# SeanNaren/deepspeech.pytorch

Measured on NVIDIA H100. Metric: utterances/sec (train step, 161x1000 spectrogram), higher is better.
Workload: dtype fp16-operands(rnn)+tf32(conv/fc)

## Files before the change

deepspeech.pytorch_b200/_lib.py:

```python
import ctypes as C
import os

_HERE = os.path.dirname(os.path.abspath(__file__))
LIB_PATH = os.path.join(_HERE, "libds2_b200.so")

RNN_LSTM, RNN_GRU, RNN_TANH = 0, 1, 2
PREC_FP32, PREC_TF32, PREC_F16 = 0, 1, 2

vp, i32, i64, f32, sz = C.c_void_p, C.c_int, C.c_int64, C.c_float, C.c_size_t


class RnnDesc(C.Structure):
    _fields_ = [("rnn_type", i32), ("bidirectional", i32), ("T", i32), ("B", i32), ("In", i32), ("H", i32),
                ("training", i32), ("bn_momentum", f32), ("bn_eps", f32), ("deferred_dw", i32)]


PROTOTYPES = {
    "ds2_version": (C.c_char_p, []),
    "ds2_last_error": (C.c_char_p, []),
    "ds2_device_check": (i32, [C.POINTER(i32)] * 3),
    "ds2_set_precision": (i32, [i32]),
    "ds2_get_precision": (i32, []),
    "ds2_launch_count": (i64, [i32]),
    "ds2_fallback_count": (i64, [i32]),
    "ds2_set_side_stream": (i32, [vp]),
    "ds2_join_side_stream": (i32, [vp]),
    "ds2_prof_enable": (i32, [i32]),
    "ds2_prof_report": (i32, [C.c_char_p, sz]),
    "ds2_seq_lens_host": (i32, [vp, i32, vp]),
    "ds2_conv_frontend_workspace_bytes": (sz, [i32, i32]),
    "ds2_conv_frontend_fwd": (i32, [i32, i32] + [vp] * 14 + [i32, f32, f32] + [vp] * 6 + [sz, vp]),
    "ds2_conv_frontend_bwd": (i32, [i32, i32] + [vp] * 22 + [sz, vp]),
    "ds2_rnn_reserve_floats": (sz, [C.POINTER(RnnDesc)]),
    "ds2_rnn_workspace_bytes": (sz, [C.POINTER(RnnDesc)]),
    "ds2_rnn_layer_fwd": (i32, [C.POINTER(RnnDesc)] + [vp] * 17 + [sz, vp]),
    "ds2_rnn_layer_bwd": (i32, [C.POINTER(RnnDesc)] + [vp] * 18 + [sz, vp]),
    "ds2_lookahead_fwd": (i32, [i32] * 4 + [vp] * 4),
    "ds2_lookahead_bwd": (i32, [i32] * 4 + [vp] * 7),
    "ds2_fc_head_workspace_bytes": (sz, [i32, i32, i32]),
    "ds2_fc_head_fwd": (i32, [i32, i32, i32] + [vp] * 6 + [i32, f32, f32, i32] + [vp] * 4 + [sz, vp]),
    "ds2_fc_head_bwd": (i32, [i32, i32, i32] + [vp] * 11 + [sz, vp]),
    "ds2_ctc_workspace_bytes": (sz, [i32, i32, i32, i32]),
    "ds2_ctc_loss_fwd_bwd": (i32, [i32, i32, i32] + [vp] * 4 + [i32, i32] + [vp] * 3 + [sz, vp]),
    "ds2_greedy_decode": (i32, [i32, i32, i32, vp, vp, i32, vp, vp, vp, vp]),
    "ds2_spectrogram_workspace_bytes": (sz, [i32]),
    "ds2_spectrogram_batch": (i32, [i32, vp, vp, vp, i32, i32, i32, vp, i32, i32, vp, i32, vp, sz, vp]),
    "ds2_spec_augment_workspace_bytes": (sz, [i32]),
    "ds2_spec_augment": (i32, [i32, i32, i32] + [vp] * 5 + [sz, vp]),
    "ds2_optim_workspace_bytes": (sz, []),
    "ds2_adamw_step": (i32, [i64] + [vp] * 4 + [f32] * 5 + [i32, f32, f32, vp, vp, vp]),
    "ds2_sgd_nesterov_step": (i32, [i64] + [vp] * 3 + [f32] * 3 + [i32, f32, f32, vp, vp, vp]),
    "ds2_gemm_workspace_bytes": (sz, [i32] * 5),
    "ds2_gemm": (i32, [i32] * 5 + [f32, vp, i32, vp, i32, f32, vp, i32, vp, sz, vp]),
    "ds2_gemm_f16": (i32, [i32] * 3 + [f32, vp, i32, vp, i32, f32, vp, i32, vp]),
}

_lib = None


class Ds2Error(RuntimeError):
    pass


def get_lib():
    global _lib
    if _lib is None:
        if not os.path.exists(LIB_PATH):
            raise Ds2Error(f"{LIB_PATH} not found: build it with `make -C deepspeech.pytorch_b200/csrc` "
                           "(or __graft_entry__.build()); there is no CPU / eager fallback")
        import torch
        lib = C.CDLL(LIB_PATH)
        for name, (res, args) in PROTOTYPES.items():
            fn = getattr(lib, name)
            fn.restype, fn.argtypes = res, args
        _lib = lib
    return _lib


def check(rc, what=""):
    if rc != 0:
        msg = get_lib().ds2_last_error().decode(errors="replace")
        raise Ds2Error(f"{what} failed with code {rc}: {msg}")


def ptr(t):
    return None if t is None else C.c_void_p(t.data_ptr())


def ptr_array(tensors):
    arr = (C.c_void_p * len(tensors))(*[None if t is None else t.data_ptr() for t in tensors])
    return arr
```

deepspeech.pytorch_b200/csrc/gemm_simt.cu:

```cuda
#include "common.cuh"

namespace ds2 {

constexpr int BM = 128, BN = 128, BK = 16, TM = 8, TN = 8;

template <bool TA, bool TB>
__global__ void __launch_bounds__(256) gemm_simt_kernel(int M, int N, int K, float alpha,
                                                        const float* __restrict__ A, int lda,
                                                        const float* __restrict__ B, int ldb, float beta,
                                                        float* __restrict__ C, int ldc, int k_per_split,
                                                        float* __restrict__ part) {
  __shared__ __align__(16) float As[BK][BM + 4];
  __shared__ __align__(16) float Bs[BK][BN + 4];
  const int tid = threadIdx.x;
  const int m0 = blockIdx.y * BM, n0 = blockIdx.x * BN;
  const int tx = tid % 16, ty = tid / 16;
  float acc[TM][TN];
#pragma unroll
  for (int i = 0; i < TM; ++i)
#pragma unroll
    for (int j = 0; j < TN; ++j) acc[i][j] = 0.f;

  const int k_begin = blockIdx.z * k_per_split;
  const int k_end = min(K, k_begin + k_per_split);
// ... 85 lines not shown
  const int kps = cdiv(cdiv(K, splits), BK) * BK, gz = cdiv(K, kps);
  if (gz > 1) *k_per_split = kps;
  return gz;
}
size_t gemm_simt_workspace_bytes(int M, int N, int K) {
  int kps;
  const int gz = simt_splits(M, N, K, &kps);
  return gz > 1 ? (size_t)gz * M * N * sizeof(float) : 0;
}

int gemm_simt(int transA, int transB, int M, int N, int K, float alpha, const float* A, int lda, const float* B,
              int ldb, float beta, float* C, int ldc, cudaStream_t st, void* ws, size_t ws_bytes) {
  if (M <= 0 || N <= 0) return DS2_OK;
  dim3 grid(cdiv(N, BN), cdiv(M, BM));
  int k_per_split;
  const int gz = simt_splits(M, N, K, &k_per_split);
  float* part = nullptr;
  if (gz > 1 && ws && ws_bytes >= (size_t)gz * M * N * sizeof(float)) {
    grid.z = gz;
    part = static_cast<float*>(ws);
  } else {
    k_per_split = K > 0 ? K : 1;
  }
  if (transA) {
    if (transB) DS2_LAUNCH((gemm_simt_kernel<true, true>), grid, 256, 0, st, M, N, K, alpha, A, lda, B, ldb, beta, C, ldc, k_per_split, part);
    else DS2_LAUNCH((gemm_simt_kernel<true, false>), grid, 256, 0, st, M, N, K, alpha, A, lda, B, ldb, beta, C, ldc, k_per_split, part);
  } else {
    if (transB) DS2_LAUNCH((gemm_simt_kernel<false, true>), grid, 256, 0, st, M, N, K, alpha, A, lda, B, ldb, beta, C, ldc, k_per_split, part);
    else DS2_LAUNCH((gemm_simt_kernel<false, false>), grid, 256, 0, st, M, N, K, alpha, A, lda, B, ldb, beta, C, ldc, k_per_split, part);
  }
  if (part) DS2_LAUNCH(sum_splits_kernel, cdiv((long long)M * N, 256), 256, 0, st, M, N, gz, part, beta, C, ldc);
  return DS2_OK;
}

}

extern "C" {
size_t ds2_gemm_workspace_bytes(int transA, int transB, int M, int N, int K) {
  const size_t tc = ds2::gemm_tc_workspace_bytes(transA, transB, M, N, K), simt = ds2::gemm_simt_workspace_bytes(M, N, K);
  return tc > simt ? tc : simt;
}

int ds2_gemm(int transA, int transB, int M, int N, int K, float alpha, const float* A, int lda, const float* B,
             int ldb, float beta, float* C, int ldc, void* ws, size_t ws_bytes, void* stream) {
  DS2_REQUIRE(M >= 0 && N >= 0 && K >= 0 && A && B && C, "ds2_gemm: bad arguments");
  cudaStream_t st = ds2::as_stream(stream);
  if (ds2::tensor_core_mode()) {
    int r = ds2::gemm_tc(transA, transB, M, N, K, alpha, A, lda, B, ldb, beta, C, ldc, ws, ws_bytes, st);
    if (r <= 0) return r;
  }
  return ds2::gemm_simt(transA, transB, M, N, K, alpha, A, lda, B, ldb, beta, C, ldc, st, ws, ws_bytes);
}

int ds2_gemm_f16(int M, int N, int K, float alpha, const void* A16, int lda, const void* B16, int ldb, float beta,
                 float* C, int ldc, void* stream) {
  DS2_REQUIRE(M > 0 && N > 0 && K > 0 && A16 && B16 && C, "ds2_gemm_f16: bad arguments");
  int r = ds2::gemm_tc_f16(M, N, K, alpha, A16, lda, B16, ldb, beta, C, ldc, nullptr, ds2::as_stream(stream));
  DS2_REQUIRE(r != 1, "ds2_gemm_f16: shape %dx%dx%d / alignment not eligible for the fp16 tensor-core kernel", M, N, K);
  return r;
}
}
```

deepspeech.pytorch_b200/csrc/gemm_tc.cu:

```cuda
#include <stdio.h>
#include <stdlib.h>

#include "common.cuh"
#include "tc_common.cuh"

namespace ds2 {

typedef CUresult (*EncodeTiledFn)(CUtensorMap*, CUtensorMapDataType, cuuint32_t, void*, const cuuint64_t*,
                                  const cuuint64_t*, const cuuint32_t*, const cuuint32_t*, CUtensorMapInterleave,
                                  CUtensorMapSwizzle, CUtensorMapL2promotion, CUtensorMapFloatOOBfill);
static EncodeTiledFn g_encode = nullptr;
static CUtensorMapDataType g_tmap_dtype = CU_TENSOR_MAP_DATA_TYPE_TFLOAT32;

static int load_encode() {
  if (g_encode) return DS2_OK;
  void* fn = nullptr;
  cudaDriverEntryPointQueryResult q;
  DS2_CHECK_CUDA(cudaGetDriverEntryPoint("cuTensorMapEncodeTiled", &fn, cudaEnableDefault, &q));
  if (!fn || q != cudaDriverEntryPointSuccess) {
    set_error("cuTensorMapEncodeTiled not available from the driver");
    return DS2_ERR_CUDA;
  }
  const char* e = getenv("DS2_TMAP_TF32");
  if (e && e[0] == '0') g_tmap_dtype = CU_TENSOR_MAP_DATA_TYPE_FLOAT32;
// ... 55 lines not shown
  if (rc) return rc;
  cuuint64_t gdim[5], gstr[4];
  cuuint32_t bx[5], estr[5];
  for (int i = 0; i < rank; ++i) { gdim[i] = dims[i]; bx[i] = box[i]; estr[i] = 1; }
  for (int i = 0; i + 1 < rank; ++i) gstr[i] = strides_bytes[i];
  CUresult r = g_encode(out, g_tmap_dtype, (cuuint32_t)rank, const_cast<float*>(base), gdim, gstr, bx, estr,
                        CU_TENSOR_MAP_INTERLEAVE_NONE, CU_TENSOR_MAP_SWIZZLE_128B, CU_TENSOR_MAP_L2_PROMOTION_L2_256B,
                        CU_TENSOR_MAP_FLOAT_OOB_FILL_NONE);
  if (r != CUDA_SUCCESS) {
    set_error("cuTensorMapEncodeTiled(rank %d) failed: %d", rank, (int)r);
    return DS2_ERR_CUDA;
  }
  return DS2_OK;
}

int make_tmap_4d_f32(CUtensorMap* out, const float* base, const unsigned long long dims[4],
                     const unsigned long long strides_bytes[3], const unsigned int box[4]) {
  int rc = load_encode();
  if (rc) return rc;
  cuuint64_t gdim[4] = {dims[0], dims[1], dims[2], dims[3]};
  cuuint64_t gstr[3] = {strides_bytes[0], strides_bytes[1], strides_bytes[2]};
  cuuint32_t bx[4] = {box[0], box[1], box[2], box[3]};
  cuuint32_t estr[4] = {1, 1, 1, 1};
  CUresult r = g_encode(out, g_tmap_dtype, 4, const_cast<float*>(base), gdim, gstr, bx, estr,
                        CU_TENSOR_MAP_INTERLEAVE_NONE, CU_TENSOR_MAP_SWIZZLE_128B, CU_TENSOR_MAP_L2_PROMOTION_L2_256B,
                        CU_TENSOR_MAP_FLOAT_OOB_FILL_NONE);
  if (r != CUDA_SUCCESS) {
    set_error("cuTensorMapEncodeTiled(4d %llu,%llu,%llu,%llu) failed: %d", dims[0], dims[1], dims[2], dims[3], (int)r);
    return DS2_ERR_CUDA;
  }
  return DS2_OK;
}

int make_tmap_f16(CUtensorMap* out, const void* base, int rank, int d0, int d1, int d2, size_t stride1,
                  size_t stride2, int box0, int box1, int box2) {
  int rc = load_encode();
  if (rc) return rc;
  cuuint64_t gdim[3] = {(cuuint64_t)d0, (cuuint64_t)d1, (cuuint64_t)d2};
  cuuint64_t gstr[2] = {(cuuint64_t)stride1 * 2, (cuuint64_t)stride2 * 2};
  cuuint32_t box[3] = {(cuuint32_t)box0, (cuuint32_t)box1, (cuuint32_t)box2};
  cuuint32_t estr[3] = {1, 1, 1};
  CUresult r = g_encode(out, CU_TENSOR_MAP_DATA_TYPE_FLOAT16, (cuuint32_t)rank, const_cast<void*>(base), gdim, gstr,
                        box, estr, CU_TENSOR_MAP_INTERLEAVE_NONE, CU_TENSOR_MAP_SWIZZLE_128B,
                        CU_TENSOR_MAP_L2_PROMOTION_L2_256B, CU_TENSOR_MAP_FLOAT_OOB_FILL_NONE);
  if (r != CUDA_SUCCESS) {
    set_error("cuTensorMapEncodeTiled(f16 rank %d dims %d,%d,%d box %d,%d,%d) failed: %d", rank, d0, d1, d2, box0, box1,
              box2, (int)r);
    return DS2_ERR_CUDA;
  }
  return DS2_OK;
}

namespace gtc {
constexpr int BM = 128, BN = 128, BK = 32, THREADS = 384, STAGES = 6;
constexpr int A_BYTES = BM * 128, B_BYTES = BN * 128, STAGE_BYTES = A_BYTES + B_BYTES;
constexpr int SMEM_BYTES = STAGES * STAGE_BYTES + 1024  + 256 ;
}

template <bool F16>
__global__ void __launch_bounds__(gtc::THREADS, 1)
gemm_tc_kernel(const __grid_constant__ CUtensorMap tmA, const __grid_constant__ CUtensorMap tmB, int M, int N, int K,
               float alpha, float beta, float* __restrict__ C, int ldc, const float* __restrict__ alpha_dev) {
  using namespace gtc;
  using namespace tc;
  constexpr int BK = F16 ? 2 * gtc::BK : gtc::BK;
  if (alpha_dev) alpha *= __ldg(alpha_dev);
  extern __shared__ uint8_t smem_raw[];
  uint8_t* smem = smem_raw + ((1024u - (smem_u32(smem_raw) & 1023u)) & 1023u);
  uint64_t* full = reinterpret_cast<uint64_t*>(smem + STAGES * STAGE_BYTES);
  uint64_t* empty = full + STAGES;
  const int warp = threadIdx.x / 32, lane = threadIdx.x % 32;
  const int m0 = blockIdx.y * BM, n0 = blockIdx.x * BN;
  const int nk_all = (K + BK - 1) / BK, per = (nk_all + (int)gridDim.z - 1) / (int)gridDim.z;
  const int kb0 = (int)blockIdx.z * per, kb1 = min(nk_all, kb0 + per), nk = max(0, kb1 - kb0);
  const bool split = gridDim.z > 1;

  if (warp == 0 && lane == 0) {
    tma_prefetch_desc(&tmA);
    tma_prefetch_desc(&tmB);
    for (int i = 0; i < STAGES; ++i) { mbar_init(&full[i], 1); mbar_init(&empty[i], 2); }
    fence_barrier_init();
  }
  __syncthreads();

  if (warp == 0) {
    if (lane == 0) {
      for (int it = 0; it < nk; ++it) {
        const int kb = kb0 + it, s = it % STAGES;
        const uint32_t ph = (it / STAGES) & 1;
        mbar_wait(&empty[s], ph ^ 1);
        mbar_arrive_expect_tx(&full[s], STAGE_BYTES);
        uint8_t* sa = smem + s * STAGE_BYTES;
        tma_load_2d(sa, &tmA, &full[s], kb * BK, m0);
        tma_load_2d(sa + A_BYTES, &tmB, &full[s], kb * BK, n0);
      }
    }
  } else if (warp >= 4) {
    const int wg = warp / 4 - 1;
    float acc[64];
#pragma unroll
    for (int i = 0; i < 64; ++i) acc[i] = 0.f;
    for (int it = 0; it < nk; ++it) {
      const int s = it % STAGES;
      mbar_wait(&full[s], (it / STAGES) & 1);
      const uint64_t adesc = smem_desc_sw128(smem_u32(smem + s * STAGE_BYTES)) + (uint64_t)(512 * wg);
      const uint64_t bdesc = smem_desc_sw128(smem_u32(smem + s * STAGE_BYTES + A_BYTES));
      wg_fence();
#pragma unroll
      for (int k = 0; k < 4; ++k)
        Wgmma<BN, F16>::mma(acc, adesc + 2 * k, bdesc + 2 * k, 1u);
      wg_release(&empty[s]);
    }
    if (nk > 0) {
      const int w = warp % 4;
      const bool vec_ok = ((ldc & 1) == 0) && ((reinterpret_cast<uintptr_t>(C) & 7) == 0);
#pragma unroll
      for (int hh = 0; hh < 2; ++hh) {
        const int row = m0 + 64 * wg + 16 * w + (lane >> 2) + 8 * hh;
        if (row >= M) continue;
        float* crow = C + (size_t)row * ldc;
#pragma unroll
        for (int i = 0; i < BN / 8; ++i) {
          const int col = n0 + 8 * i + 2 * (lane & 3);
          float2 o = make_float2(alpha * acc[4 * i + 2 * hh], alpha * acc[4 * i + 2 * hh + 1]);
          if (vec_ok && col + 1 < N) {
            float2* cp2 = reinterpret_cast<float2*>(crow + col);
            if (split) {
              atomicAdd(cp2, o);
            } else {
              if (beta != 0.f) {
                const float2 old = *cp2;
                o.x = fmaf(beta, old.x, o.x);
                o.y = fmaf(beta, old.y, o.y);
              }
              *cp2 = o;
            }
          } else {
#pragma unroll
            for (int j = 0; j < 2; ++j) {
              if (col + j >= N) break;
              float v = j ? o.y : o.x;
              if (split) {
                atomicAdd(crow + col + j, v);
              } else {
                if (beta != 0.f) v = fmaf(beta, crow[col + j], v);
                crow[col + j] = v;
              }
            }
          }
        }
      }
    }
  }
}

__global__ void transpose_strided_kernel(int R, int C, const float* __restrict__ in, size_t ldi,
                                         float* __restrict__ out, size_t ldo) {
  __shared__ float tile[32][33];
  int c = blockIdx.x * 32 + threadIdx.x, r0 = blockIdx.y * 32;
  for (int j = threadIdx.y; j < 32; j += 8)
    if (r0 + j < R && c < C) tile[j][threadIdx.x] = in[(size_t)(r0 + j) * ldi + c];
  __syncthreads();
  int r = r0 + threadIdx.x, c0 = blockIdx.x * 32;
  for (int j = threadIdx.y; j < 32; j += 8)
    if (c0 + j < C && r < R) out[(size_t)(c0 + j) * ldo + r] = tile[threadIdx.x][j];
}

int transpose_strided(int R, int C, const float* in, size_t ldi, float* out, size_t ldo, cudaStream_t st) {
  DS2_LAUNCH(transpose_strided_kernel, dim3(cdiv(C, 32), cdiv(R, 32)), dim3(32, 8), 0, st, R, C, in, ldi, out, ldo);
  return DS2_OK;
}
int transpose(int R, int C, const float* in, float* out, cudaStream_t st) {
  return transpose_strided(R, C, in, (size_t)C, out, (size_t)R, st);
}

static inline size_t k4(int K) { return (size_t)((K + 3) / 4 * 4); }

size_t gemm_tc_workspace_bytes(int transA, int transB, int M, int N, int K) {
  size_t n = 0;
  if (transA) n += align_up((size_t)M * k4(K) * 4, 256);
  if (!transB) n += align_up((size_t)N * k4(K) * 4, 256);
  return n;
}

static bool tc_eligible(int M, int N, int K) { return K >= 32 && M >= 32 && N >= 16 && (long long)M * N * K >= (1 << 18); }

static int choose_splits(const char* env, float beta) {
  const char* e = getenv(env);
  const int forced = e ? atoi(e) : 0;
  if (forced >= 2 && forced <= 3 && (beta == 0.f || beta == 1.f)) return 1 << (forced - 1);
  return 1;
}

template <bool F16>
static int launch_gemm_tc(const CUtensorMap& tmA, const CUtensorMap& tmB, int M, int N, int K, float alpha, float beta,
                          float* C, int ldc, int splits, cudaStream_t st, const float* alpha_dev = nullptr) {
  auto kern = gemm_tc_kernel<F16>;
  static DeviceOnce attr_once;
  if (attr_once.first()) {
    DS2_CHECK_CUDA(cudaFuncSetAttribute(kern, cudaFuncAttributeMaxDynamicSharedMemorySize, gtc::SMEM_BYTES));
    attr_once.done();
  }
  if (splits > 1 && beta == 0.f)
    DS2_CHECK_CUDA(cudaMemset2DAsync(C, (size_t)ldc * sizeof(float), 0, (size_t)N * sizeof(float), (size_t)M, st));
  dim3 grid(cdiv(N, gtc::BN), cdiv(M, gtc::BM), splits);
  DS2_LAUNCH(kern, grid, gtc::THREADS, gtc::SMEM_BYTES, st, tmA, tmB, M, N, K, alpha, beta, C, ldc, alpha_dev);
  return DS2_OK;
}

int gemm_tc(int transA, int transB, int M, int N, int K, float alpha, const float* A, int lda, const float* B,
            int ldb, float beta, float* C, int ldc, void* ws, size_t ws_bytes, cudaStream_t st) {
  if (!tc_eligible(M, N, K)) return 1;
  Arena ar(ws, ws_bytes);
  const float* Ak = A;
  int ldak = lda;
  if (transA) {
    float* t = ar.take<float>((size_t)M * k4(K));
    if (!t) return 1;
    int rc = transpose_strided(K, M, A, (size_t)lda, t, k4(K), st);
    if (rc) return rc;
    Ak = t;
    ldak = (int)k4(K);
  }
  const float* Bk = B;
  int ldbk = ldb;
  if (!transB) {
    float* t = ar.take<float>((size_t)N * k4(K));
    if (!t) return 1;
    int rc = transpose_strided(K, N, B, (size_t)ldb, t, k4(K), st);
    if (rc) return rc;
    Bk = t;
    ldbk = (int)k4(K);
  }
  if ((ldak & 3) || (ldbk & 3) || (reinterpret_cast<uintptr_t>(Ak) & 15) || (reinterpret_cast<uintptr_t>(Bk) & 15))
    return 1;
  const int splits = choose_splits("DS2_GEMM_CFG", beta);
  CUtensorMap tmA, tmB;
  int rc = make_tmap_2d(&tmA, Ak, M, K, ldak, gtc::BM, gtc::BK);
  if (rc) return rc;
  rc = make_tmap_2d(&tmB, Bk, N, K, ldbk, gtc::BN, gtc::BK);
  if (rc) return rc;
  return launch_gemm_tc<false>(tmA, tmB, M, N, K, alpha, beta, C, ldc, splits, st);
}

int gemm_tc_f16(int M, int N, int K, float alpha, const void* A16, int lda, const void* B16, int ldb, float beta,
                float* C, int ldc, const float* alpha_dev, cudaStream_t st) {
  if (!tc_eligible(M, N, K) || M < 128) return 1;
  if ((lda & 7) || (ldb & 7) || (reinterpret_cast<uintptr_t>(A16) & 15) || (reinterpret_cast<uintptr_t>(B16) & 15)) return 1;
  const int splits = choose_splits("DS2_GEMM16_CFG", beta);
  CUtensorMap tmA, tmB;
  int rc = make_tmap_f16(&tmA, A16, 2, K, M, 1, (size_t)lda, 0, 64, gtc::BM, 1);
  if (rc) return rc;
  rc = make_tmap_f16(&tmB, B16, 2, K, N, 1, (size_t)ldb, 0, 64, gtc::BN, 1);
  if (rc) return rc;
  return launch_gemm_tc<true>(tmA, tmB, M, N, K, alpha, beta, C, ldc, splits, st, alpha_dev);
}

}
```

deepspeech.pytorch_b200/csrc/tc_common.cuh:

```cuda
#pragma once
#include <cuda.h>
#include <cuda_runtime.h>
#include <stdint.h>

#include <type_traits>

#include "wgmma.cuh"

namespace ds2 {
namespace tc {

__device__ __forceinline__ uint32_t smem_u32(const void* p) { return (uint32_t)__cvta_generic_to_shared(p); }

__device__ __forceinline__ void mbar_init(uint64_t* bar, uint32_t count) {
  asm volatile("mbarrier.init.shared::cta.b64 [%0], %1;" ::"r"(smem_u32(bar)), "r"(count));
}
__device__ __forceinline__ void fence_barrier_init() { asm volatile("fence.mbarrier_init.release.cluster;" ::: "memory"); }
__device__ __forceinline__ void fence_proxy_async() { asm volatile("fence.proxy.async.shared::cta;" ::: "memory"); }
__device__ __forceinline__ void mbar_arrive_expect_tx(uint64_t* bar, uint32_t bytes) {
  asm volatile("mbarrier.arrive.expect_tx.shared::cta.b64 _, [%0], %1;" ::"r"(smem_u32(bar)), "r"(bytes) : "memory");
}
__device__ __forceinline__ void mbar_arrive(uint64_t* bar) {
  asm volatile("mbarrier.arrive.shared::cta.b64 _, [%0];" ::"r"(smem_u32(bar)) : "memory");
}
// ... 25 lines not shown
}

__device__ __forceinline__ void tma_prefetch_desc(const CUtensorMap* m) {
  asm volatile("prefetch.tensormap [%0];" ::"l"(reinterpret_cast<uint64_t>(m)) : "memory");
}
__device__ __forceinline__ void tma_load_2d(void* smem_dst, const CUtensorMap* m, uint64_t* bar, int c0, int c1) {
  asm volatile(
      "cp.async.bulk.tensor.2d.shared::cluster.global.tile.mbarrier::complete_tx::bytes [%0], [%1, {%3, %4}], [%2];"
      ::"r"(smem_u32(smem_dst)), "l"(reinterpret_cast<uint64_t>(m)), "r"(smem_u32(bar)), "r"(c0), "r"(c1)
      : "memory");
}
__device__ __forceinline__ void tma_load_3d(void* smem_dst, const CUtensorMap* m, uint64_t* bar, int c0, int c1,
                                            int c2) {
  asm volatile(
      "cp.async.bulk.tensor.3d.shared::cluster.global.tile.mbarrier::complete_tx::bytes [%0], [%1, {%3, %4, %5}], [%2];"
      ::"r"(smem_u32(smem_dst)), "l"(reinterpret_cast<uint64_t>(m)), "r"(smem_u32(bar)), "r"(c0), "r"(c1), "r"(c2)
      : "memory");
}

__device__ __forceinline__ void mbar_arrive_expect_tx_w(uint64_t* bar, uint32_t bytes) {
  asm volatile(
      "{\n\t.reg .pred pe;\n\telect.sync _|pe, 0xffffffff;\n\t"
      "@pe mbarrier.arrive.expect_tx.shared::cta.b64 _, [%0], %1;\n\t}" ::"r"(smem_u32(bar)), "r"(bytes)
      : "memory");
}
__device__ __forceinline__ void tma_load_2d_w(void* smem_dst, const CUtensorMap* m, uint64_t* bar, int c0, int c1) {
  asm volatile(
      "{\n\t.reg .pred pe;\n\telect.sync _|pe, 0xffffffff;\n\t"
      "@pe cp.async.bulk.tensor.2d.shared::cluster.global.tile.mbarrier::complete_tx::bytes [%0], [%1, {%3, %4}], [%2];\n\t}"
      ::"r"(smem_u32(smem_dst)), "l"(reinterpret_cast<uint64_t>(m)), "r"(smem_u32(bar)), "r"(c0), "r"(c1)
      : "memory");
}
__device__ __forceinline__ void tma_load_3d_w(void* smem_dst, const CUtensorMap* m, uint64_t* bar, int c0, int c1,
                                              int c2) {
  asm volatile(
      "{\n\t.reg .pred pe;\n\telect.sync _|pe, 0xffffffff;\n\t"
      "@pe cp.async.bulk.tensor.3d.shared::cluster.global.tile.mbarrier::complete_tx::bytes [%0], [%1, {%3, %4, %5}], [%2];\n\t}"
      ::"r"(smem_u32(smem_dst)), "l"(reinterpret_cast<uint64_t>(m)), "r"(smem_u32(bar)), "r"(c0), "r"(c1), "r"(c2)
      : "memory");
}

__device__ __forceinline__ uint64_t smem_desc_sw128(uint32_t smem_addr) {
  uint64_t d = 0;
  d |= (uint64_t)((smem_addr & 0x3FFFF) >> 4);
  d |= (uint64_t)1 << 16;
  d |= (uint64_t)(1024 >> 4) << 32;
  d |= (uint64_t)1 << 62;
  return d;
}
__device__ __forceinline__ void wg_fence() { asm volatile("wgmma.fence.sync.aligned;" ::: "memory"); }
__device__ __forceinline__ void wg_commit() { asm volatile("wgmma.commit_group.sync.aligned;" ::: "memory"); }
template <int N>
__device__ __forceinline__ void wg_wait() { asm volatile("wgmma.wait_group.sync.aligned %0;" ::"n"(N) : "memory"); }
__device__ __forceinline__ uint64_t warp_uniform(uint64_t v) {
  const uint32_t lo = __shfl_sync(0xffffffffu, (uint32_t)v, 0), hi = __shfl_sync(0xffffffffu, (uint32_t)(v >> 32), 0);
  return ((uint64_t)hi << 32) | lo;
}
__device__ __forceinline__ void wg_release(uint64_t* bar) {
  wg_commit();
  wg_wait<0>();
  if ((threadIdx.x & 127) == 0) mbar_arrive(bar);
}

__host__ __device__ constexpr int acc_pitch(int NB) { return (NB + 31) / 32 * 32 + 1; }
__host__ __device__ constexpr int acc_image_bytes(int NB) { return 128 * acc_pitch(NB) * 4; }

__device__ __forceinline__ void wg_release_all(uint64_t* bar) {
  wg_commit();
  wg_wait<0>();
  mbar_arrive(bar);
}

template <int MH, int NCH>
struct WgAcc {
  float r[MH][NCH][16];
};
template <bool F16, int MH, int NCH>
__device__ __forceinline__ void wg_mma_nb(WgAcc<MH, NCH>& acc, uint64_t adesc, uint64_t bdesc, uint32_t accumulate) {
#pragma unroll
  for (int h = 0; h < MH; ++h) {
#pragma unroll
    for (int c = 0; c < NCH; ++c)
      Wgmma<32, F16>::mma(acc.r[h][c], adesc + (uint64_t)(512 * h), bdesc + (uint64_t)(256 * c), accumulate);
  }
}
template <bool F16, int MH, int NCH>
__device__ __forceinline__ void wg_mma4(WgAcc<MH, NCH>& acc, uint64_t adesc, uint64_t bdesc, uint32_t accumulate) {
  wg_fence();
  wg_mma_nb<F16>(acc, adesc, bdesc, accumulate);
#pragma unroll
  for (int k = 1; k < 4; ++k) wg_mma_nb<F16>(acc, adesc + 2 * k, bdesc + 2 * k, 1u);
}
template <int MAXCH, class F>
__device__ __forceinline__ void with_nch(int NB, F&& f) {
  if (NB == 32) f(std::integral_constant<int, 1>{});
  else if constexpr (MAXCH >= 2) {
    if (NB == 64) f(std::integral_constant<int, 2>{});
    else if constexpr (MAXCH >= 4) {
      if (NB == 96) f(std::integral_constant<int, 3>{});
      else if (NB == 128) f(std::integral_constant<int, 4>{});
    }
  }
}
template <int MH, int NCH>
__device__ __forceinline__ void wg_store_acc(const WgAcc<MH, NCH>& acc, float* tm, int pitch) {
  const int w = (threadIdx.x >> 5) & 3, l = threadIdx.x & 31;
// ... 41 lines not shown
```

deepspeech.pytorch_b200/csrc/wgmma.cuh:

```cuda
#pragma once
#include <stdint.h>

namespace ds2 {
namespace tc {

template <int N, bool F16>
struct Wgmma;

template <>
struct Wgmma<8, false> {
  __device__ __forceinline__ static void mma(float* d, uint64_t a, uint64_t b, uint32_t acc) {
    asm volatile(
        "{\n\t.reg .pred p;\n\tsetp.ne.b32 p, %6, 0;\n\t"
        "wgmma.mma_async.sync.aligned.m64n8k8.f32.tf32.tf32 {%0, %1, %2, %3}, %4, %5, p, 1, 1;\n\t}"
        : "+f"(d[0]), "+f"(d[1]), "+f"(d[2]), "+f"(d[3])
        : "l"(a), "l"(b), "r"(acc));
  }
};

template <>
struct Wgmma<8, true> {
  __device__ __forceinline__ static void mma(float* d, uint64_t a, uint64_t b, uint32_t acc) {
    asm volatile(
        "{\n\t.reg .pred p;\n\tsetp.ne.b32 p, %6, 0;\n\t"
// ... 85 lines not shown
  __device__ __forceinline__ static void mma(float* d, uint64_t a, uint64_t b, uint32_t acc) {
    asm volatile(
        "{\n\t.reg .pred p;\n\tsetp.ne.b32 p, %50, 0;\n\t"
        "wgmma.mma_async.sync.aligned.m64n96k16.f32.f16.f16 {%0, %1, %2, %3, %4, %5, %6, %7, %8, %9, %10, %11, %12, %13, %14, %15, %16, %17, %18, %19, %20, %21, %22, %23, %24, %25, %26, %27, %28, %29, %30, %31, %32, %33, %34, %35, %36, %37, %38, %39, %40, %41, %42, %43, %44, %45, %46, %47}, %48, %49, p, 1, 1, 0, 0;\n\t}"
        : "+f"(d[0]), "+f"(d[1]), "+f"(d[2]), "+f"(d[3]), "+f"(d[4]), "+f"(d[5]), "+f"(d[6]), "+f"(d[7]), "+f"(d[8]), "+f"(d[9]), "+f"(d[10]), "+f"(d[11]), "+f"(d[12]), "+f"(d[13]), "+f"(d[14]), "+f"(d[15]), "+f"(d[16]), "+f"(d[17]), "+f"(d[18]), "+f"(d[19]), "+f"(d[20]), "+f"(d[21]), "+f"(d[22]), "+f"(d[23]), "+f"(d[24]), "+f"(d[25]), "+f"(d[26]), "+f"(d[27]), "+f"(d[28]), "+f"(d[29]), "+f"(d[30]), "+f"(d[31]), "+f"(d[32]), "+f"(d[33]), "+f"(d[34]), "+f"(d[35]), "+f"(d[36]), "+f"(d[37]), "+f"(d[38]), "+f"(d[39]), "+f"(d[40]), "+f"(d[41]), "+f"(d[42]), "+f"(d[43]), "+f"(d[44]), "+f"(d[45]), "+f"(d[46]), "+f"(d[47])
        : "l"(a), "l"(b), "r"(acc));
  }
};

template <>
struct Wgmma<128, false> {
  __device__ __forceinline__ static void mma(float* d, uint64_t a, uint64_t b, uint32_t acc) {
    asm volatile(
        "{\n\t.reg .pred p;\n\tsetp.ne.b32 p, %66, 0;\n\t"
        "wgmma.mma_async.sync.aligned.m64n128k8.f32.tf32.tf32 {%0, %1, %2, %3, %4, %5, %6, %7, %8, %9, %10, %11, %12, %13, %14, %15, %16, %17, %18, %19, %20, %21, %22, %23, %24, %25, %26, %27, %28, %29, %30, %31, %32, %33, %34, %35, %36, %37, %38, %39, %40, %41, %42, %43, %44, %45, %46, %47, %48, %49, %50, %51, %52, %53, %54, %55, %56, %57, %58, %59, %60, %61, %62, %63}, %64, %65, p, 1, 1;\n\t}"
        : "+f"(d[0]), "+f"(d[1]), "+f"(d[2]), "+f"(d[3]), "+f"(d[4]), "+f"(d[5]), "+f"(d[6]), "+f"(d[7]), "+f"(d[8]), "+f"(d[9]), "+f"(d[10]), "+f"(d[11]), "+f"(d[12]), "+f"(d[13]), "+f"(d[14]), "+f"(d[15]), "+f"(d[16]), "+f"(d[17]), "+f"(d[18]), "+f"(d[19]), "+f"(d[20]), "+f"(d[21]), "+f"(d[22]), "+f"(d[23]), "+f"(d[24]), "+f"(d[25]), "+f"(d[26]), "+f"(d[27]), "+f"(d[28]), "+f"(d[29]), "+f"(d[30]), "+f"(d[31]), "+f"(d[32]), "+f"(d[33]), "+f"(d[34]), "+f"(d[35]), "+f"(d[36]), "+f"(d[37]), "+f"(d[38]), "+f"(d[39]), "+f"(d[40]), "+f"(d[41]), "+f"(d[42]), "+f"(d[43]), "+f"(d[44]), "+f"(d[45]), "+f"(d[46]), "+f"(d[47]), "+f"(d[48]), "+f"(d[49]), "+f"(d[50]), "+f"(d[51]), "+f"(d[52]), "+f"(d[53]), "+f"(d[54]), "+f"(d[55]), "+f"(d[56]), "+f"(d[57]), "+f"(d[58]), "+f"(d[59]), "+f"(d[60]), "+f"(d[61]), "+f"(d[62]), "+f"(d[63])
        : "l"(a), "l"(b), "r"(acc));
  }
};

template <>
struct Wgmma<128, true> {
  __device__ __forceinline__ static void mma(float* d, uint64_t a, uint64_t b, uint32_t acc) {
    asm volatile(
        "{\n\t.reg .pred p;\n\tsetp.ne.b32 p, %66, 0;\n\t"
        "wgmma.mma_async.sync.aligned.m64n128k16.f32.f16.f16 {%0, %1, %2, %3, %4, %5, %6, %7, %8, %9, %10, %11, %12, %13, %14, %15, %16, %17, %18, %19, %20, %21, %22, %23, %24, %25, %26, %27, %28, %29, %30, %31, %32, %33, %34, %35, %36, %37, %38, %39, %40, %41, %42, %43, %44, %45, %46, %47, %48, %49, %50, %51, %52, %53, %54, %55, %56, %57, %58, %59, %60, %61, %62, %63}, %64, %65, p, 1, 1, 0, 0;\n\t}"
        : "+f"(d[0]), "+f"(d[1]), "+f"(d[2]), "+f"(d[3]), "+f"(d[4]), "+f"(d[5]), "+f"(d[6]), "+f"(d[7]), "+f"(d[8]), "+f"(d[9]), "+f"(d[10]), "+f"(d[11]), "+f"(d[12]), "+f"(d[13]), "+f"(d[14]), "+f"(d[15]), "+f"(d[16]), "+f"(d[17]), "+f"(d[18]), "+f"(d[19]), "+f"(d[20]), "+f"(d[21]), "+f"(d[22]), "+f"(d[23]), "+f"(d[24]), "+f"(d[25]), "+f"(d[26]), "+f"(d[27]), "+f"(d[28]), "+f"(d[29]), "+f"(d[30]), "+f"(d[31]), "+f"(d[32]), "+f"(d[33]), "+f"(d[34]), "+f"(d[35]), "+f"(d[36]), "+f"(d[37]), "+f"(d[38]), "+f"(d[39]), "+f"(d[40]), "+f"(d[41]), "+f"(d[42]), "+f"(d[43]), "+f"(d[44]), "+f"(d[45]), "+f"(d[46]), "+f"(d[47]), "+f"(d[48]), "+f"(d[49]), "+f"(d[50]), "+f"(d[51]), "+f"(d[52]), "+f"(d[53]), "+f"(d[54]), "+f"(d[55]), "+f"(d[56]), "+f"(d[57]), "+f"(d[58]), "+f"(d[59]), "+f"(d[60]), "+f"(d[61]), "+f"(d[62]), "+f"(d[63])
        : "l"(a), "l"(b), "r"(acc));
  }
};

template <>
struct Wgmma<176, false> {
  __device__ __forceinline__ static void mma(float* d, uint64_t a, uint64_t b, uint32_t acc) {
    asm volatile(
        "{\n\t.reg .pred p;\n\tsetp.ne.b32 p, %90, 0;\n\t"
        "wgmma.mma_async.sync.aligned.m64n176k8.f32.tf32.tf32 {%0, %1, %2, %3, %4, %5, %6, %7, %8, %9, %10, %11, %12, %13, %14, %15, %16, %17, %18, %19, %20, %21, %22, %23, %24, %25, %26, %27, %28, %29, %30, %31, %32, %33, %34, %35, %36, %37, %38, %39, %40, %41, %42, %43, %44, %45, %46, %47, %48, %49, %50, %51, %52, %53, %54, %55, %56, %57, %58, %59, %60, %61, %62, %63, %64, %65, %66, %67, %68, %69, %70, %71, %72, %73, %74, %75, %76, %77, %78, %79, %80, %81, %82, %83, %84, %85, %86, %87}, %88, %89, p, 1, 1;\n\t}"
        : "+f"(d[0]), "+f"(d[1]), "+f"(d[2]), "+f"(d[3]), "+f"(d[4]), "+f"(d[5]), "+f"(d[6]), "+f"(d[7]), "+f"(d[8]), "+f"(d[9]), "+f"(d[10]), "+f"(d[11]), "+f"(d[12]), "+f"(d[13]), "+f"(d[14]), "+f"(d[15]), "+f"(d[16]), "+f"(d[17]), "+f"(d[18]), "+f"(d[19]), "+f"(d[20]), "+f"(d[21]), "+f"(d[22]), "+f"(d[23]), "+f"(d[24]), "+f"(d[25]), "+f"(d[26]), "+f"(d[27]), "+f"(d[28]), "+f"(d[29]), "+f"(d[30]), "+f"(d[31]), "+f"(d[32]), "+f"(d[33]), "+f"(d[34]), "+f"(d[35]), "+f"(d[36]), "+f"(d[37]), "+f"(d[38]), "+f"(d[39]), "+f"(d[40]), "+f"(d[41]), "+f"(d[42]), "+f"(d[43]), "+f"(d[44]), "+f"(d[45]), "+f"(d[46]), "+f"(d[47]), "+f"(d[48]), "+f"(d[49]), "+f"(d[50]), "+f"(d[51]), "+f"(d[52]), "+f"(d[53]), "+f"(d[54]), "+f"(d[55]), "+f"(d[56]), "+f"(d[57]), "+f"(d[58]), "+f"(d[59]), "+f"(d[60]), "+f"(d[61]), "+f"(d[62]), "+f"(d[63]), "+f"(d[64]), "+f"(d[65]), "+f"(d[66]), "+f"(d[67]), "+f"(d[68]), "+f"(d[69]), "+f"(d[70]), "+f"(d[71]), "+f"(d[72]), "+f"(d[73]), "+f"(d[74]), "+f"(d[75]), "+f"(d[76]), "+f"(d[77]), "+f"(d[78]), "+f"(d[79]), "+f"(d[80]), "+f"(d[81]), "+f"(d[82]), "+f"(d[83]), "+f"(d[84]), "+f"(d[85]), "+f"(d[86]), "+f"(d[87])
        : "l"(a), "l"(b), "r"(acc));
  }
};

template <>
struct Wgmma<176, true> {
  __device__ __forceinline__ static void mma(float* d, uint64_t a, uint64_t b, uint32_t acc) {
    asm volatile(
        "{\n\t.reg .pred p;\n\tsetp.ne.b32 p, %90, 0;\n\t"
        "wgmma.mma_async.sync.aligned.m64n176k16.f32.f16.f16 {%0, %1, %2, %3, %4, %5, %6, %7, %8, %9, %10, %11, %12, %13, %14, %15, %16, %17, %18, %19, %20, %21, %22, %23, %24, %25, %26, %27, %28, %29, %30, %31, %32, %33, %34, %35, %36, %37, %38, %39, %40, %41, %42, %43, %44, %45, %46, %47, %48, %49, %50, %51, %52, %53, %54, %55, %56, %57, %58, %59, %60, %61, %62, %63, %64, %65, %66, %67, %68, %69, %70, %71, %72, %73, %74, %75, %76, %77, %78, %79, %80, %81, %82, %83, %84, %85, %86, %87}, %88, %89, p, 1, 1, 0, 0;\n\t}"
        : "+f"(d[0]), "+f"(d[1]), "+f"(d[2]), "+f"(d[3]), "+f"(d[4]), "+f"(d[5]), "+f"(d[6]), "+f"(d[7]), "+f"(d[8]), "+f"(d[9]), "+f"(d[10]), "+f"(d[11]), "+f"(d[12]), "+f"(d[13]), "+f"(d[14]), "+f"(d[15]), "+f"(d[16]), "+f"(d[17]), "+f"(d[18]), "+f"(d[19]), "+f"(d[20]), "+f"(d[21]), "+f"(d[22]), "+f"(d[23]), "+f"(d[24]), "+f"(d[25]), "+f"(d[26]), "+f"(d[27]), "+f"(d[28]), "+f"(d[29]), "+f"(d[30]), "+f"(d[31]), "+f"(d[32]), "+f"(d[33]), "+f"(d[34]), "+f"(d[35]), "+f"(d[36]), "+f"(d[37]), "+f"(d[38]), "+f"(d[39]), "+f"(d[40]), "+f"(d[41]), "+f"(d[42]), "+f"(d[43]), "+f"(d[44]), "+f"(d[45]), "+f"(d[46]), "+f"(d[47]), "+f"(d[48]), "+f"(d[49]), "+f"(d[50]), "+f"(d[51]), "+f"(d[52]), "+f"(d[53]), "+f"(d[54]), "+f"(d[55]), "+f"(d[56]), "+f"(d[57]), "+f"(d[58]), "+f"(d[59]), "+f"(d[60]), "+f"(d[61]), "+f"(d[62]), "+f"(d[63]), "+f"(d[64]), "+f"(d[65]), "+f"(d[66]), "+f"(d[67]), "+f"(d[68]), "+f"(d[69]), "+f"(d[70]), "+f"(d[71]), "+f"(d[72]), "+f"(d[73]), "+f"(d[74]), "+f"(d[75]), "+f"(d[76]), "+f"(d[77]), "+f"(d[78]), "+f"(d[79]), "+f"(d[80]), "+f"(d[81]), "+f"(d[82]), "+f"(d[83]), "+f"(d[84]), "+f"(d[85]), "+f"(d[86]), "+f"(d[87])
        : "l"(a), "l"(b), "r"(acc));
  }
};

}
}
```

include/ds2_b200.h:

```cpp
#ifndef DS2_B200_H_
#define DS2_B200_H_

#include <stddef.h>
#include <stdint.h>

#ifdef __cplusplus
extern "C" {
#endif

#define DS2_OK                 0
#define DS2_ERR_INVALID       -1
#define DS2_ERR_CUDA          -2
#define DS2_ERR_UNSORTED      -3
#define DS2_ERR_WORKSPACE     -4

enum { DS2_RNN_LSTM = 0, DS2_RNN_GRU = 1, DS2_RNN_TANH = 2 };
enum { DS2_PREC_FP32 = 0, DS2_PREC_TF32 = 1, DS2_PREC_F16 = 2 };

#define DS2_NUM_FREQ   161
#define DS2_CONV_CH     32
#define DS2_CONV1_D     81
#define DS2_CONV2_D     41
#define DS2_RNN_IN0   1312

// ... 63 lines not shown
                      float* dz, float* dx, float* dw, void* stream);

size_t ds2_fc_head_workspace_bytes(int rows, int H, int C);
int ds2_fc_head_fwd(int rows, int H, int C, const float* x, const float* bn_gamma, const float* bn_beta,
                    float* bn_rmean, float* bn_rvar, const float* w, int training, float momentum, float eps,
                    int softmax, float* logits, float* xhat, float* stats,
                    void* workspace, size_t workspace_bytes, void* stream);
int ds2_fc_head_bwd(int rows, int H, int C, const float* bn_gamma, const float* bn_beta, const float* w,
                    const float* xhat,
                    const float* stats, const float* dlogits, float* dx, float* dbn_gamma, float* dbn_beta,
                    float* dw, void* workspace, size_t workspace_bytes, void* stream);

size_t ds2_ctc_workspace_bytes(int T, int B, int C, int max_tgt_len);
int ds2_ctc_loss_fwd_bwd(int T, int B, int C, const float* logits, const int64_t* targets,
                         const int32_t* in_len, const int32_t* tgt_len, int max_tgt_len, int blank,
                         float* nll, float* grad, void* workspace, size_t workspace_bytes, void* stream);

int ds2_greedy_decode(int B, int T, int C, const float* probs, const int32_t* out_len, int blank,
                      int32_t* labels, int32_t* offsets, int32_t* counts, void* stream);

size_t ds2_optim_workspace_bytes(void);
int ds2_adamw_step(int64_t n, float* p, const float* g, float* m, float* v, float lr, float beta1, float beta2,
                   float eps, float weight_decay, int step, float grad_scale, float max_norm,
                   float* grad_norm_out, void* norm_ws, void* stream);
int ds2_sgd_nesterov_step(int64_t n, float* p, const float* g, float* momentum_buf, float lr, float momentum,
                          float weight_decay, int first_step, float grad_scale, float max_norm,
                          float* grad_norm_out, void* norm_ws, void* stream);

size_t ds2_spectrogram_workspace_bytes(int n_utts);
int ds2_spectrogram_batch(int n_utts, const float* wave, const int64_t* offsets, const int32_t* dst_row,
                          int max_samples, int n_fft, int hop, const float* window, int pad_reflect, int normalize,
                          float* out, int Tmax, void* workspace, size_t workspace_bytes, void* stream);

typedef struct {
  int32_t idx;
  int32_t d;
  int32_t f0, f;
  int32_t t0, t;
  float Z[9];
  int32_t reserved;
} Ds2SpecAugDraws;

size_t ds2_spec_augment_workspace_bytes(int n_utts);
int ds2_spec_augment(int n_utts, int F, int Tmax, const float* in, const int32_t* frames,
                     const Ds2SpecAugDraws* draws, float* out, void* workspace, size_t workspace_bytes, void* stream);

size_t ds2_gemm_workspace_bytes(int transA, int transB, int M, int N, int K);
int ds2_gemm(int transA, int transB, int M, int N, int K, float alpha, const float* A, int lda,
             const float* B, int ldb, float beta, float* C, int ldc,
             void* workspace, size_t workspace_bytes, void* stream);

int ds2_gemm_f16(int M, int N, int K, float alpha, const void* A16, int lda, const void* B16, int ldb, float beta,
                 float* C, int ldc, void* stream);

#ifdef __cplusplus
}
#endif
#endif
```

Measured before the change: 586.1.

## Add BN=256 wgmma tiles, register rebalancing, and async wgmma pipelining to TC GEMM

Makes the TMA/wgmma GEMM kernel templated on the N tile, choosing a 128x256 tile with 4 stages when N exceeds 128, and adds m64n256 wgmma variants for tf32 and f16. Producer warps give up registers via setmaxnreg so the consumer warpgroups can hold the larger accumulator. Stage release now lags one iteration, using wgmma commit/wait<1> so consecutive MMAs overlap instead of fully draining each stage. It also exposes a device-side alpha scaling entry point. The larger tiles cut operand reloads but reduce pipeline depth and grid size for mid-sized N.

```diff
diff --git a/deepspeech.pytorch_b200/_lib.py b/deepspeech.pytorch_b200/_lib.py
--- a/deepspeech.pytorch_b200/_lib.py
+++ b/deepspeech.pytorch_b200/_lib.py
@@ -53,6 +53,7 @@
     "ds2_gemm_workspace_bytes": (sz, [i32] * 5),
     "ds2_gemm": (i32, [i32] * 5 + [f32, vp, i32, vp, i32, f32, vp, i32, vp, sz, vp]),
     "ds2_gemm_f16": (i32, [i32] * 3 + [f32, vp, i32, vp, i32, f32, vp, i32, vp]),
+    "ds2_gemm_f16_scaled": (i32, [i32] * 3 + [f32, vp, i32, vp, i32, f32, vp, i32, vp, vp]),
 }
 
 _lib = None
diff --git a/deepspeech.pytorch_b200/csrc/gemm_simt.cu b/deepspeech.pytorch_b200/csrc/gemm_simt.cu
--- a/deepspeech.pytorch_b200/csrc/gemm_simt.cu
+++ b/deepspeech.pytorch_b200/csrc/gemm_simt.cu
@@ -161,11 +161,16 @@
   return ds2::gemm_simt(transA, transB, M, N, K, alpha, A, lda, B, ldb, beta, C, ldc, st, ws, ws_bytes);
 }
 
-int ds2_gemm_f16(int M, int N, int K, float alpha, const void* A16, int lda, const void* B16, int ldb, float beta,
-                 float* C, int ldc, void* stream) {
+int ds2_gemm_f16_scaled(int M, int N, int K, float alpha, const void* A16, int lda, const void* B16, int ldb,
+                        float beta, float* C, int ldc, const float* alpha_dev, void* stream) {
   DS2_REQUIRE(M > 0 && N > 0 && K > 0 && A16 && B16 && C, "ds2_gemm_f16: bad arguments");
-  int r = ds2::gemm_tc_f16(M, N, K, alpha, A16, lda, B16, ldb, beta, C, ldc, nullptr, ds2::as_stream(stream));
+  int r = ds2::gemm_tc_f16(M, N, K, alpha, A16, lda, B16, ldb, beta, C, ldc, alpha_dev, ds2::as_stream(stream));
   DS2_REQUIRE(r != 1, "ds2_gemm_f16: shape %dx%dx%d / alignment not eligible for the fp16 tensor-core kernel", M, N, K);
   return r;
 }
+
+int ds2_gemm_f16(int M, int N, int K, float alpha, const void* A16, int lda, const void* B16, int ldb, float beta,
+                 float* C, int ldc, void* stream) {
+  return ds2_gemm_f16_scaled(M, N, K, alpha, A16, lda, B16, ldb, beta, C, ldc, nullptr, stream);
 }
+}
diff --git a/deepspeech.pytorch_b200/csrc/gemm_tc.cu b/deepspeech.pytorch_b200/csrc/gemm_tc.cu
--- a/deepspeech.pytorch_b200/csrc/gemm_tc.cu
+++ b/deepspeech.pytorch_b200/csrc/gemm_tc.cu
@@ -131,17 +131,24 @@
 }
 
 namespace gtc {
-constexpr int BM = 128, BN = 128, BK = 32, THREADS = 384, STAGES = 6;
-constexpr int A_BYTES = BM * 128, B_BYTES = BN * 128, STAGE_BYTES = A_BYTES + B_BYTES;
-constexpr int SMEM_BYTES = STAGES * STAGE_BYTES + 1024  + 256 ;
-}
-
-template <bool F16>
+constexpr int BM = 128, BK = 32, THREADS = 384;
+constexpr int PRODUCER_REGS = 40, MMA_REGS = 232;
+template <int BN>
+struct Cfg {
+  static constexpr int STAGES = BN == 256 ? 4 : 6;
+  static constexpr int A_BYTES = BM * 128, B_BYTES = BN * 128, STAGE_BYTES = A_BYTES + B_BYTES;
+  static constexpr int SMEM_BYTES = STAGES * STAGE_BYTES + 1024  + 256 ;
+};
+static_assert(Cfg<256>::SMEM_BYTES <= 227 * 1024 && Cfg<128>::SMEM_BYTES <= 227 * 1024, "shared memory");
+}
+
+template <bool F16, int BN>
 __global__ void __launch_bounds__(gtc::THREADS, 1)
 gemm_tc_kernel(const __grid_constant__ CUtensorMap tmA, const __grid_constant__ CUtensorMap tmB, int M, int N, int K,
                float alpha, float beta, float* __restrict__ C, int ldc, const float* __restrict__ alpha_dev) {
   using namespace gtc;
   using namespace tc;
+  constexpr int STAGES = Cfg<BN>::STAGES, A_BYTES = Cfg<BN>::A_BYTES, STAGE_BYTES = Cfg<BN>::STAGE_BYTES;
   constexpr int BK = F16 ? 2 * gtc::BK : gtc::BK;
   if (alpha_dev) alpha *= __ldg(alpha_dev);
   extern __shared__ uint8_t smem_raw[];
@@ -162,8 +169,9 @@
   }
   __syncthreads();
 
-  if (warp == 0) {
-    if (lane == 0) {
+  if (warp < 4) {
+    setmaxnreg_dec<PRODUCER_REGS>();
+    if (warp == 0 && lane == 0) {
       for (int it = 0; it < nk; ++it) {
         const int kb = kb0 + it, s = it % STAGES;
         const uint32_t ph = (it / STAGES) & 1;
@@ -174,11 +182,13 @@
         tma_load_2d(sa + A_BYTES, &tmB, &full[s], kb * BK, n0);
       }
     }
-  } else if (warp >= 4) {
+  } else {
+    setmaxnreg_inc<MMA_REGS>();
     const int wg = warp / 4 - 1;
-    float acc[64];
-#pragma unroll
-    for (int i = 0; i < 64; ++i) acc[i] = 0.f;
+    const bool leader = (threadIdx.x & 127) == 0;
+    float acc[BN / 2];
+#pragma unroll
+    for (int i = 0; i < BN / 2; ++i) acc[i] = 0.f;
     for (int it = 0; it < nk; ++it) {
       const int s = it % STAGES;
       mbar_wait(&full[s], (it / STAGES) & 1);
@@ -188,8 +198,12 @@
 #pragma unroll
       for (int k = 0; k < 4; ++k)
         Wgmma<BN, F16>::mma(acc, adesc + 2 * k, bdesc + 2 * k, 1u);
-      wg_release(&empty[s]);
+      wg_commit();
+      wg_wait<1>();
+      if (it > 0 && leader) mbar_arrive(&empty[(it - 1) % STAGES]);
     }
+    wg_wait<0>();
+    if (nk > 0 && leader) mbar_arrive(&empty[(nk - 1) % STAGES]);
     if (nk > 0) {
       const int w = warp % 4;
       const bool vec_ok = ((ldc & 1) == 0) && ((reinterpret_cast<uintptr_t>(C) & 7) == 0);
@@ -271,20 +285,30 @@
   return 1;
 }
 
+static int tile_n(int N) { return N > 128 ? 256 : 128; }
+
+template <bool F16, int BN>
+static int launch_gemm_tc(const CUtensorMap& tmA, const CUtensorMap& tmB, int M, int N, int K, float alpha, float beta,
+                          float* C, int ldc, int splits, cudaStream_t st, const float* alpha_dev) {
+  auto kern = gemm_tc_kernel<F16, BN>;
+  constexpr int smem = gtc::Cfg<BN>::SMEM_BYTES;
+  static DeviceOnce attr_once;
+  if (attr_once.first()) {
+    DS2_CHECK_CUDA(cudaFuncSetAttribute(kern, cudaFuncAttributeMaxDynamicSharedMemorySize, smem));
+    attr_once.done();
+  }
+  if (splits > 1 && beta == 0.f)
+    DS2_CHECK_CUDA(cudaMemset2DAsync(C, (size_t)ldc * sizeof(float), 0, (size_t)N * sizeof(float), (size_t)M, st));
+  dim3 grid(cdiv(N, BN), cdiv(M, gtc::BM), splits);
+  DS2_LAUNCH(kern, grid, gtc::THREADS, smem, st, tmA, tmB, M, N, K, alpha, beta, C, ldc, alpha_dev);
+  return DS2_OK;
+}
+
 template <bool F16>
 static int launch_gemm_tc(const CUtensorMap& tmA, const CUtensorMap& tmB, int M, int N, int K, float alpha, float beta,
                           float* C, int ldc, int splits, cudaStream_t st, const float* alpha_dev = nullptr) {
-  auto kern = gemm_tc_kernel<F16>;
-  static DeviceOnce attr_once;
-  if (attr_once.first()) {
-    DS2_CHECK_CUDA(cudaFuncSetAttribute(kern, cudaFuncAttributeMaxDynamicSharedMemorySize, gtc::SMEM_BYTES));
-    attr_once.done();
-  }
-  if (splits > 1 && beta == 0.f)
-    DS2_CHECK_CUDA(cudaMemset2DAsync(C, (size_t)ldc * sizeof(float), 0, (size_t)N * sizeof(float), (size_t)M, st));
-  dim3 grid(cdiv(N, gtc::BN), cdiv(M, gtc::BM), splits);
-  DS2_LAUNCH(kern, grid, gtc::THREADS, gtc::SMEM_BYTES, st, tmA, tmB, M, N, K, alpha, beta, C, ldc, alpha_dev);
-  return DS2_OK;
+  if (tile_n(N) == 256) return launch_gemm_tc<F16, 256>(tmA, tmB, M, N, K, alpha, beta, C, ldc, splits, st, alpha_dev);
+  return launch_gemm_tc<F16, 128>(tmA, tmB, M, N, K, alpha, beta, C, ldc, splits, st, alpha_dev);
 }
 
 int gemm_tc(int transA, int transB, int M, int N, int K, float alpha, const float* A, int lda, const float* B,
@@ -317,7 +341,7 @@
   CUtensorMap tmA, tmB;
   int rc = make_tmap_2d(&tmA, Ak, M, K, ldak, gtc::BM, gtc::BK);
   if (rc) return rc;
-  rc = make_tmap_2d(&tmB, Bk, N, K, ldbk, gtc::BN, gtc::BK);
+  rc = make_tmap_2d(&tmB, Bk, N, K, ldbk, tile_n(N), gtc::BK);
   if (rc) return rc;
   return launch_gemm_tc<false>(tmA, tmB, M, N, K, alpha, beta, C, ldc, splits, st);
 }
@@ -330,7 +354,7 @@
   CUtensorMap tmA, tmB;
   int rc = make_tmap_f16(&tmA, A16, 2, K, M, 1, (size_t)lda, 0, 64, gtc::BM, 1);
   if (rc) return rc;
-  rc = make_tmap_f16(&tmB, B16, 2, K, N, 1, (size_t)ldb, 0, 64, gtc::BN, 1);
+  rc = make_tmap_f16(&tmB, B16, 2, K, N, 1, (size_t)ldb, 0, 64, tile_n(N), 1);
   if (rc) return rc;
   return launch_gemm_tc<true>(tmA, tmB, M, N, K, alpha, beta, C, ldc, splits, st, alpha_dev);
 }
diff --git a/deepspeech.pytorch_b200/csrc/tc_common.cuh b/deepspeech.pytorch_b200/csrc/tc_common.cuh
--- a/deepspeech.pytorch_b200/csrc/tc_common.cuh
+++ b/deepspeech.pytorch_b200/csrc/tc_common.cuh
@@ -101,6 +101,10 @@
 __device__ __forceinline__ void wg_commit() { asm volatile("wgmma.commit_group.sync.aligned;" ::: "memory"); }
 template <int N>
 __device__ __forceinline__ void wg_wait() { asm volatile("wgmma.wait_group.sync.aligned %0;" ::"n"(N) : "memory"); }
+template <int N>
+__device__ __forceinline__ void setmaxnreg_dec() { asm volatile("setmaxnreg.dec.sync.aligned.u32 %0;" ::"n"(N)); }
+template <int N>
+__device__ __forceinline__ void setmaxnreg_inc() { asm volatile("setmaxnreg.inc.sync.aligned.u32 %0;" ::"n"(N)); }
 __device__ __forceinline__ uint64_t warp_uniform(uint64_t v) {
   const uint32_t lo = __shfl_sync(0xffffffffu, (uint32_t)v, 0), hi = __shfl_sync(0xffffffffu, (uint32_t)(v >> 32), 0);
   return ((uint64_t)hi << 32) | lo;
diff --git a/deepspeech.pytorch_b200/csrc/wgmma.cuh b/deepspeech.pytorch_b200/csrc/wgmma.cuh
--- a/deepspeech.pytorch_b200/csrc/wgmma.cuh
+++ b/deepspeech.pytorch_b200/csrc/wgmma.cuh
@@ -161,5 +161,27 @@
   }
 };
 
+template <>
+struct Wgmma<256, false> {
+  __device__ __forceinline__ static void mma(float* d, uint64_t a, uint64_t b, uint32_t acc) {
+    asm volatile(
+        "{\n\t.reg .pred p;\n\tsetp.ne.b32 p, %130, 0;\n\t"
+        "wgmma.mma_async.sync.aligned.m64n256k8.f32.tf32.tf32 {%0, %1, %2, %3, %4, %5, %6, %7, %8, %9, %10, %11, %12, %13, %14, %15, %16, %17, %18, %19, %20, %21, %22, %23, %24, %25, %26, %27, %28, %29, %30, %31, %32, %33, %34, %35, %36, %37, %38, %39, %40, %41, %42, %43, %44, %45, %46, %47, %48, %49, %50, %51, %52, %53, %54, %55, %56, %57, %58, %59, %60, %61, %62, %63, %64, %65, %66, %67, %68, %69, %70, %71, %72, %73, %74, %75, %76, %77, %78, %79, %80, %81, %82, %83, %84, %85, %86, %87, %88, %89, %90, %91, %92, %93, %94, %95, %96, %97, %98, %99, %100, %101, %102, %103, %104, %105, %106, %107, %108, %109, %110, %111, %112, %113, %114, %115, %116, %117, %118, %119, %120, %121, %122, %123, %124, %125, %126, %127}, %128, %129, p, 1, 1;\n\t}"
+        : "+f"(d[0]), "+f"(d[1]), "+f"(d[2]), "+f"(d[3]), "+f"(d[4]), "+f"(d[5]), "+f"(d[6]), "+f"(d[7]), "+f"(d[8]), "+f"(d[9]), "+f"(d[10]), "+f"(d[11]), "+f"(d[12]), "+f"(d[13]), "+f"(d[14]), "+f"(d[15]), "+f"(d[16]), "+f"(d[17]), "+f"(d[18]), "+f"(d[19]), "+f"(d[20]), "+f"(d[21]), "+f"(d[22]), "+f"(d[23]), "+f"(d[24]), "+f"(d[25]), "+f"(d[26]), "+f"(d[27]), "+f"(d[28]), "+f"(d[29]), "+f"(d[30]), "+f"(d[31]), "+f"(d[32]), "+f"(d[33]), "+f"(d[34]), "+f"(d[35]), "+f"(d[36]), "+f"(d[37]), "+f"(d[38]), "+f"(d[39]), "+f"(d[40]), "+f"(d[41]), "+f"(d[42]), "+f"(d[43]), "+f"(d[44]), "+f"(d[45]), "+f"(d[46]), "+f"(d[47]), "+f"(d[48]), "+f"(d[49]), "+f"(d[50]), "+f"(d[51]), "+f"(d[52]), "+f"(d[53]), "+f"(d[54]), "+f"(d[55]), "+f"(d[56]), "+f"(d[57]), "+f"(d[58]), "+f"(d[59]), "+f"(d[60]), "+f"(d[61]), "+f"(d[62]), "+f"(d[63]), "+f"(d[64]), "+f"(d[65]), "+f"(d[66]), "+f"(d[67]), "+f"(d[68]), "+f"(d[69]), "+f"(d[70]), "+f"(d[71]), "+f"(d[72]), "+f"(d[73]), "+f"(d[74]), "+f"(d[75]), "+f"(d[76]), "+f"(d[77]), "+f"(d[78]), "+f"(d[79]), "+f"(d[80]), "+f"(d[81]), "+f"(d[82]), "+f"(d[83]), "+f"(d[84]), "+f"(d[85]), "+f"(d[86]), "+f"(d[87]), "+f"(d[88]), "+f"(d[89]), "+f"(d[90]), "+f"(d[91]), "+f"(d[92]), "+f"(d[93]), "+f"(d[94]), "+f"(d[95]), "+f"(d[96]), "+f"(d[97]), "+f"(d[98]), "+f"(d[99]), "+f"(d[100]), "+f"(d[101]), "+f"(d[102]), "+f"(d[103]), "+f"(d[104]), "+f"(d[105]), "+f"(d[106]), "+f"(d[107]), "+f"(d[108]), "+f"(d[109]), "+f"(d[110]), "+f"(d[111]), "+f"(d[112]), "+f"(d[113]), "+f"(d[114]), "+f"(d[115]), "+f"(d[116]), "+f"(d[117]), "+f"(d[118]), "+f"(d[119]), "+f"(d[120]), "+f"(d[121]), "+f"(d[122]), "+f"(d[123]), "+f"(d[124]), "+f"(d[125]), "+f"(d[126]), "+f"(d[127])
+        : "l"(a), "l"(b), "r"(acc));
+  }
+};
+
+template <>
+struct Wgmma<256, true> {
+  __device__ __forceinline__ static void mma(float* d, uint64_t a, uint64_t b, uint32_t acc) {
+    asm volatile(
+        "{\n\t.reg .pred p;\n\tsetp.ne.b32 p, %130, 0;\n\t"
+        "wgmma.mma_async.sync.aligned.m64n256k16.f32.f16.f16 {%0, %1, %2, %3, %4, %5, %6, %7, %8, %9, %10, %11, %12, %13, %14, %15, %16, %17, %18, %19, %20, %21, %22, %23, %24, %25, %26, %27, %28, %29, %30, %31, %32, %33, %34, %35, %36, %37, %38, %39, %40, %41, %42, %43, %44, %45, %46, %47, %48, %49, %50, %51, %52, %53, %54, %55, %56, %57, %58, %59, %60, %61, %62, %63, %64, %65, %66, %67, %68, %69, %70, %71, %72, %73, %74, %75, %76, %77, %78, %79, %80, %81, %82, %83, %84, %85, %86, %87, %88, %89, %90, %91, %92, %93, %94, %95, %96, %97, %98, %99, %100, %101, %102, %103, %104, %105, %106, %107, %108, %109, %110, %111, %112, %113, %114, %115, %116, %117, %118, %119, %120, %121, %122, %123, %124, %125, %126, %127}, %128, %129, p, 1, 1, 0, 0;\n\t}"
+        : "+f"(d[0]), "+f"(d[1]), "+f"(d[2]), "+f"(d[3]), "+f"(d[4]), "+f"(d[5]), "+f"(d[6]), "+f"(d[7]), "+f"(d[8]), "+f"(d[9]), "+f"(d[10]), "+f"(d[11]), "+f"(d[12]), "+f"(d[13]), "+f"(d[14]), "+f"(d[15]), "+f"(d[16]), "+f"(d[17]), "+f"(d[18]), "+f"(d[19]), "+f"(d[20]), "+f"(d[21]), "+f"(d[22]), "+f"(d[23]), "+f"(d[24]), "+f"(d[25]), "+f"(d[26]), "+f"(d[27]), "+f"(d[28]), "+f"(d[29]), "+f"(d[30]), "+f"(d[31]), "+f"(d[32]), "+f"(d[33]), "+f"(d[34]), "+f"(d[35]), "+f"(d[36]), "+f"(d[37]), "+f"(d[38]), "+f"(d[39]), "+f"(d[40]), "+f"(d[41]), "+f"(d[42]), "+f"(d[43]), "+f"(d[44]), "+f"(d[45]), "+f"(d[46]), "+f"(d[47]), "+f"(d[48]), "+f"(d[49]), "+f"(d[50]), "+f"(d[51]), "+f"(d[52]), "+f"(d[53]), "+f"(d[54]), "+f"(d[55]), "+f"(d[56]), "+f"(d[57]), "+f"(d[58]), "+f"(d[59]), "+f"(d[60]), "+f"(d[61]), "+f"(d[62]), "+f"(d[63]), "+f"(d[64]), "+f"(d[65]), "+f"(d[66]), "+f"(d[67]), "+f"(d[68]), "+f"(d[69]), "+f"(d[70]), "+f"(d[71]), "+f"(d[72]), "+f"(d[73]), "+f"(d[74]), "+f"(d[75]), "+f"(d[76]), "+f"(d[77]), "+f"(d[78]), "+f"(d[79]), "+f"(d[80]), "+f"(d[81]), "+f"(d[82]), "+f"(d[83]), "+f"(d[84]), "+f"(d[85]), "+f"(d[86]), "+f"(d[87]), "+f"(d[88]), "+f"(d[89]), "+f"(d[90]), "+f"(d[91]), "+f"(d[92]), "+f"(d[93]), "+f"(d[94]), "+f"(d[95]), "+f"(d[96]), "+f"(d[97]), "+f"(d[98]), "+f"(d[99]), "+f"(d[100]), "+f"(d[101]), "+f"(d[102]), "+f"(d[103]), "+f"(d[104]), "+f"(d[105]), "+f"(d[106]), "+f"(d[107]), "+f"(d[108]), "+f"(d[109]), "+f"(d[110]), "+f"(d[111]), "+f"(d[112]), "+f"(d[113]), "+f"(d[114]), "+f"(d[115]), "+f"(d[116]), "+f"(d[117]), "+f"(d[118]), "+f"(d[119]), "+f"(d[120]), "+f"(d[121]), "+f"(d[122]), "+f"(d[123]), "+f"(d[124]), "+f"(d[125]), "+f"(d[126]), "+f"(d[127])
+        : "l"(a), "l"(b), "r"(acc));
+  }
+};
+
 }
 }
diff --git a/include/ds2_b200.h b/include/ds2_b200.h
--- a/include/ds2_b200.h
+++ b/include/ds2_b200.h
@@ -139,6 +139,8 @@
 
 int ds2_gemm_f16(int M, int N, int K, float alpha, const void* A16, int lda, const void* B16, int ldb, float beta,
                  float* C, int ldc, void* stream);
+int ds2_gemm_f16_scaled(int M, int N, int K, float alpha, const void* A16, int lda, const void* B16, int ldb,
+                        float beta, float* C, int ldc, const float* alpha_dev, void* stream);
 
 #ifdef __cplusplus
 }
```

Measured after the change: 610.6 (median of 6 runs). 4.2% higher.
